# ZhaoyangLyu/Point_Diffusion_Refinement

Measured on AMD Instinct MI355X. Metric: DDPM reverse steps/sec (T=1000, N=2048), higher is better.
Workload: dtype f32; 1 GPU; BASELINE configs[1]: B=32/GPU, N=2048, 3072-pt mirrored condition, T=1000 DDPM reverse sampling, random-init dual-path PointNet++ (9.76 M params), cached condition step; global_batch=32, parallelism=dp1, launch=hipGraph replay, noise=device Philox, execution=fused channel-last HIP

## Files before the change

### point_diffusion_refinement_amd/csrc/ball_query.hip

```cpp
#include "pdr_common.h"

namespace {

template <int NCH, bool RESIDENT>
__global__ __launch_bounds__(256) void ball_query_kernel(
    const float* __restrict__ new_xyz, const float* __restrict__ xyz, int n, int m,
    float radius2, int nsample, int qpw, int* __restrict__ idx,
    int* __restrict__ counts) {
  const int b = blockIdx.y;
  const int lane = threadIdx.x & 63;
  const int wave = __builtin_amdgcn_readfirstlane(threadIdx.x >> 6);
  const float* p = xyz + static_cast<size_t>(b) * n * 3;
  const float* q = new_xyz + static_cast<size_t>(b) * m * 3;
  int* oi = idx + static_cast<size_t>(b) * m * nsample;
  int* oc = counts + static_cast<size_t>(b) * m;

  const int nch = RESIDENT ? NCH : (n + 63) / 64;
  float px[NCH], py[NCH], pz[NCH];
  if constexpr (RESIDENT) {
    if constexpr (NCH <= 32) {
#pragma unroll
      for (int c = 0; c < NCH; ++c) {
        const int k = min(c * 64 + lane, n - 1);
        px[c] = p[k * 3 + 0];
        py[c] = p[k * 3 + 1];
        pz[c] = p[k * 3 + 2];
      }
#pragma unroll
      for (int c = 0; c < NCH; ++c) {
        const bool ok = c * 64 + lane < n;
        px[c] = ok ? px[c] : __builtin_inff();
        py[c] = ok ? py[c] : __builtin_inff();
        pz[c] = ok ? pz[c] : __builtin_inff();
      }
    } else {
#pragma unroll
      for (int c = 0; c < NCH; ++c) {
        const int k = c * 64 + lane;
        const bool ok = k < n;
        px[c] = ok ? p[k * 3 + 0] : __builtin_inff();
        py[c] = ok ? p[k * 3 + 1] : __builtin_inff();
        pz[c] = ok ? p[k * 3 + 2] : __builtin_inff();
      }
    }
    __builtin_amdgcn_s_waitcnt(0x0F70);
  }

  const int j0 = (blockIdx.x * 4 + wave) * qpw;
  const int jf = min(j0, m - 1);
  float nqx = q[jf * 3 + 0], nqy = q[jf * 3 + 1], nqz = q[jf * 3 + 2];
  for (int jj = 0; jj < qpw; ++jj) {
    const int j = j0 + jj;
    if (j >= m) break;
    const float qx = nqx, qy = nqy, qz = nqz;
    {
      const int jn = min(j + 1, m - 1);
      nqx = q[jn * 3 + 0], nqy = q[jn * 3 + 1], nqz = q[jn * 3 + 2];
    }
    int* row = oi + static_cast<size_t>(j) * nsample;
    int cnt = 0;
    int first = 0;
    auto scan = [&](int c, float x, float y, float z) {
      const float dx = qx - x, dy = qy - y, dz = qz - z;
      const float d2 = PDR_SUM3(dx, dy, dz);
      const bool hit = d2 < radius2;
      const unsigned long long mask = __ballot(hit);
      if (mask != 0ull) {
        if (cnt == 0) first = c * 64 + __builtin_ctzll(mask);
        const int pos = cnt + __builtin_amdgcn_mbcnt_hi(
                                  static_cast<unsigned>(mask >> 32),
                                  __builtin_amdgcn_mbcnt_lo(static_cast<unsigned>(mask), 0u));
        if (hit && pos < nsample) row[pos] = c * 64 + lane;
        cnt += __builtin_popcountll(mask);
      }
    };
    if constexpr (RESIDENT) {
#pragma unroll
      for (int c = 0; c < NCH; ++c) {
        if (cnt < nsample) scan(c, px[c], py[c], pz[c]);
      }
    } else {
      for (int c = 0; c < nch && cnt < nsample; ++c) {
        const int k = c * 64 + lane;
        const bool ok = k < n;
        const int kc = ok ? k : n - 1;
        const float x = p[kc * 3 + 0], y = p[kc * 3 + 1], z = p[kc * 3 + 2];
        scan(c, ok ? x : __builtin_inff(), ok ? y : __builtin_inff(), ok ? z : __builtin_inff());
      }
    }
    const int filled = cnt < nsample ? cnt : nsample;
    for (int l = filled + lane; l < nsample; l += 64) row[l] = first;
    if (lane == 0) oc[j] = filled;
  }
}

struct BallPlan {
  int nch;
  int resident;
  int qpw;
  int gx;
};

int plan_ball_query(int B, int n, int m, BallPlan* p) {
  if (B < 0 || n <= 0 || m < 0) return PDR_EINVAL;
  p->nch = p->resident = p->qpw = p->gx = 0;
  if (B == 0 || m == 0) return PDR_OK;
  constexpr int kResident[] = {1, 2, 4, 8, 16, 32, 48, 64};
  p->nch = 1;
  for (const int nch : kResident)
    if (n <= 64 * nch) {
      p->nch = nch, p->resident = 1;
      break;
    }
  int qpw = 16;
  while (qpw > 1 && static_cast<long long>(B) * ((m + 4 * qpw - 1) / (4 * qpw)) < 1024) qpw >>= 1;
  p->qpw = qpw;
  p->gx = (m + 4 * qpw - 1) / (4 * qpw);
  return PDR_OK;
}

template <int NCH, bool RESIDENT>
int launch(const BallPlan& p, const float* new_xyz, const float* xyz, int B, int n, int m, float radius2,
           int nsample, int* idx, int* counts, hipStream_t s) {
  hipLaunchKernelGGL((ball_query_kernel<NCH, RESIDENT>), dim3(p.gx, B), dim3(256), 0, s, new_xyz, xyz, n,
                     m, radius2, nsample, p.qpw, idx, counts);
  return pdr::check_launch();
}

}

extern "C" int pdr_ball_query_plan(int B, int n, int m, int out[4]) {
  if (!out) return PDR_EINVAL;
  BallPlan p;
  const int rc = plan_ball_query(B, n, m, &p);
  if (rc != PDR_OK) return rc;
  out[0] = p.nch, out[1] = p.resident, out[2] = p.qpw, out[3] = p.gx;
  return PDR_OK;
}

extern "C" int pdr_ball_query(const float* new_xyz, const float* xyz, int B, int n, int m,
                              float radius, int nsample, int* idx, int* counts,
                              pdr_stream_t stream) {
  BallPlan p;
  const int rc = plan_ball_query(B, n, m, &p);
  if (rc != PDR_OK) return rc;
  if (nsample <= 0) return PDR_EINVAL;
  if (B == 0 || m == 0) return PDR_OK;
  if (!new_xyz || !xyz || !idx || !counts) return PDR_EINVAL;
  hipStream_t s = pdr::as_stream(stream);
  const float radius2 = radius * radius;
  if (!p.resident) return launch<1, false>(p, new_xyz, xyz, B, n, m, radius2, nsample, idx, counts, s);
#define PDR_BQ_CASE(NCH) \
  case NCH:              \
    return launch<NCH, true>(p, new_xyz, xyz, B, n, m, radius2, nsample, idx, counts, s)
  switch (p.nch) {
    PDR_BQ_CASE(1);
    PDR_BQ_CASE(2);
    PDR_BQ_CASE(4);
    PDR_BQ_CASE(8);
    PDR_BQ_CASE(16);
    PDR_BQ_CASE(32);
    PDR_BQ_CASE(48);
    PDR_BQ_CASE(64);
  }
#undef PDR_BQ_CASE
  return PDR_EUNSUPPORTED;
}
```

### point_diffusion_refinement_amd/pointnet2/fused_network.py

```python
import contextlib
import ctypes
from collections import namedtuple

import torch
import torch.nn as nn
import torch.nn.functional as F

from .. import _lib
from ..pointnet2_ops import _ext
from ..pointnet2_ops.attention import MyGroupNorm
from .models.pointnet2_ssg_sem import calc_t_emb


USE_SPLIT_FIRST = True
SPLIT_QUERY_CONV = True
FUSE_SCORE_POOL = True
FUSE_CONDITION_BRANCH = True
USE_VIRTUAL_FIRST = True
USE_VIRTUAL_KNN = True
GATHER_RES = 4096
GATHER_RES_KNN = True
NATIVE_EMBED = True
STEP_TABLE = True
FUSE_GLOBAL_PNET = True
# ... 1453 lines not shown
        if self.s1[0][1] is None or self.s2[0][1] is None:
            raise NotImplementedError("fused Pnet2Stage: the first layer of a stage is normalised")

    @staticmethod
    def _mlp(x, stages, B, n):
        (c1, n1), (c2, n2) = stages
        lo = run_layer(x, c1, fold=FoldReq(n1, c1.Cout, n))
        a1 = act_from(lo, c1.Cout, B * n, B, n, scale=lo.folded[0], shift=lo.folded[1], post_relu=True)
        if n2 is None:
            return act_from(run_layer(a1, c2), c2.Cout, B * n, B, n)
        lo = run_layer(a1, c2, fold=FoldReq(n2, c2.Cout, n))
        return act_from(lo, c2.Cout, B * n, B, n, scale=lo.folded[0], shift=lo.folded[1], post_relu=True)

    def __call__(self, g_in):
        B, n, _ = g_in.shape
        x = Act(feature_segments(g_in), B * n, B, n)
        f = self._mlp(x, self.s1, B, n)
        g = act_colmax(f)
        C1 = f.C
        Y, ld = f.segs[0].t, f.segs[0].ld
        dev = g.device
        one = torch.ones((B, C1), device=dev) if f.scale is None else f.scale
        zero = torch.zeros((B, C1), device=dev)
        tm = _lib.load().pdr_fused_layer_tile_rows(n, self.s2[0][0].Cout)
        d = 1
        while d * 2 <= tm and n % (d * 2) == 0 and tm % (d * 2) == 0:
            d *= 2
        if d > 1 and C1 % 4 == 0:
            second, s_second = Seg(torch.zeros((B * n // d, C1), device=dev), 0, C1, C1, d), one
        else:
            second, s_second = Seg(Y, 0, C1, ld), zero
        both = Act([Seg(Y, 0, C1, ld), second], B * n, B, n,
                   scale=torch.cat([one, s_second], 1).contiguous(),
                   shift=torch.cat([zero if f.shift is None else f.shift, zero], 1).contiguous(),
                   add=torch.cat([zero, g], 1).contiguous(), add_ld=2 * C1, post_relu=f.post_relu)
        return act_colmax(self._mlp(both, self.s2, B, n))


class FusedCloudConditionNet:

    def __init__(self, net, precision="f32"):
        hp = net.hparams
        if precision == "split_bf16":
            import warnings
            warnings.warn("precision='split_bf16' is a deprecated alias of 'split_f16' (f16 hi + lo halves; see the "
                          "range contract in include/pdr_hip.h)", DeprecationWarning, stacklevel=2)
            precision = "split_f16"
        if precision not in ("f32", "split_f16"):
            raise ValueError("precision must be 'f32' or 'split_f16'")
        self.precision = precision
        if net.scale_factor != 1:
            raise NotImplementedError("fused path: scale_factor == 1 (coordinates are not rescaled here)")
        if not (net.include_local_feature and net.include_global_feature and hp['include_class_condition']
                and net.attach_position_to_input_feature and net.bn and not hp['bn_first']
                and net.network_activation == 'relu'):
            raise NotImplementedError("configuration outside the fused family (see module docstring)")
        self.net = net
        self.bank = EmbeddingBank()
        b = self.bank
        self.enc_map = [FusedGroupedBlock(m.mapper, m.mlp, m.attention_module, b) for m in net.encoder_feature_map]
        self.dec_map = [FusedGroupedBlock(m.mapper, m.mlp, m.attention_module, b) for m in net.decoder_feature_map]
        self.sa = []
        for sa in net.SA_modules:
            if len(sa.groupers) != 1 or not sa.use_attention_module:
                raise NotImplementedError("fused path: single-scale SA with attention")
            blk = FusedGroupedBlock(sa.groupers[0], sa.mlps[0], sa.attention_modules[0], b)
            blk.npoint = sa.npoint
            self.sa.append(blk)
        self.fp = [FusedKnnFP(fp, b) for fp in net.FP_modules]
        for blk in self.enc_map + self.dec_map + self.sa:
            blk.dedup = True
        self.cond_sa = []
        for sa in net.SA_modules_condition:
            if len(sa.groupers) != 1 or not sa.use_attention_module:
                raise NotImplementedError("fused path: single-scale SA with attention")
            blk = FusedGroupedBlock(sa.groupers[0], sa.mlps[0], sa.attention_modules[0], b)
            blk.npoint = sa.npoint
            self.cond_sa.append(blk)
        self.cond_fp = [FusedKnnFP(fp, b) for fp in net.FP_modules_condition]
        head = list(net.fc_lyaer)
        if not (len(head) == 4 and isinstance(head[1], nn.GroupNorm) and isinstance(head[2], nn.ReLU)):
            raise NotImplementedError("fused path: Conv1d -> GroupNorm -> ReLU -> Conv1d head")
        self.head1, self.head_norm, self.head2 = Conv([head[0]]), Norm(head[1]), Conv([head[3]])
        b.pack()
        try:
            self.global_pnet = FusedPnet2Stage(net.global_pnet)
        except NotImplementedError:
            self.global_pnet = None
        self.enc_cl = self.dec_cl = None
        self._synced = False
        self._streams = {"side": None, "fps": None, "aux": None}
        self.return_strided_eps = False
        self.two_streams = True
        self._label_key = None
        self.dedup = True
        self.probe = None
        self.step_table = None

    def _stream_named(self, name):
        if self._streams[name] is None:
            self._streams[name] = torch.cuda.Stream(device=next(self.net.parameters()).device)
        return self._streams[name]

    def sync_condition(self):
        net = self.net

        def convert(dst, src):
            if dst is not None and len(dst) == len(src) and all(d.shape == (f.shape[0], f.shape[2], f.shape[1])
                                                                for d, f in zip(dst, src)):
                for d, f in zip(dst, src):
                    d.copy_(f.transpose(1, 2))
                return dst
            return [f.transpose(1, 2).contiguous() for f in src]

        self.enc_cl = convert(self.enc_cl, net.encoder_cond_features)
        self.dec_cl = convert(self.dec_cl, net.decoder_cond_features)
        saved_precision = _PRECISION[0]
        _PRECISION[0] = self.precision
        with torch.no_grad():
            _new_forward()
            for i, blk in enumerate(self.enc_map):
                blk.prepare_static_source(net.l_uvw[i], self.enc_cl[i])
            for i, blk in enumerate(self.dec_map):
                blk.prepare_static_source(net.l_uvw[i], self.dec_cl[i])
            _XYZ4.clear()
            self.bank.evaluate_kind("c", net.global_feature, static=True)
        _PRECISION[0] = saved_precision
        self._synced = True

    def _condition_branch(self, condition):
        net, bank = self.net, self.bank
        uvw = condition[:, :, 0:3].contiguous()
        cond0 = torch.cat([condition[:, :, 3:], uvw / net.scale_factor], dim=2).contiguous() \
            if condition.shape[2] > 3 else (uvw / net.scale_factor)
        raw = net.partial_in_fea_dim - 3 if net.attach_position_to_input_feature else net.partial_in_fea_dim
        g_in = torch.cat([uvw, condition[:, :, 3:3 + raw]], dim=2) if raw > 0 else uvw
        if self.global_pnet is not None and FUSE_GLOBAL_PNET:
            net.global_feature = self.global_pnet(g_in.contiguous())
        else:
            net.global_feature = net.global_pnet(g_in.transpose(1, 2)).detach().clone()
        l_uvw, l_cond = [uvw], [cond0]
        for i, sa in enumerate(self.cond_sa):
            sel = _ext.furthest_point_sampling(l_uvw[i], sa.npoint)
            l_uvw.append(gather_rows(l_uvw[i], sel))
            centre = gather_rows(l_cond[i], sel)
            l_cond.append(sa(l_uvw[i], l_cond[i], l_uvw[i + 1], centre, bank, subset=True))
        net.l_uvw = l_uvw
        net.encoder_cond_features = [f.transpose(1, 2).contiguous() for f in l_cond]
        for i in range(-1, -(len(self.cond_fp) + 1), -1):
            l_cond[i - 1] = self.cond_fp[i](l_uvw[i - 1], l_uvw[i], l_cond[i - 1], l_cond[i], bank)
        net.decoder_cond_features = [f.transpose(1, 2).contiguous() for f in l_cond]
        self._synced = False

    @torch.no_grad()
    def forward(self, pointcloud, condition, ts=None, label=None, use_retained_condition_feature=False):
        net, hp, bank = self.net, self.net.hparams, self.bank
        fresh = not use_retained_condition_feature or net.encoder_cond_features is None or \
            net.decoder_cond_features is None or net.global_feature is None
        if fresh:
            if not FUSE_CONDITION_BRANCH:
                out = net(pointcloud, condition, ts=ts, label=label,
                          use_retained_condition_feature=use_retained_condition_feature)
                if use_retained_condition_feature and label is not None:
                    self._refresh_class_embedding(label)
                return out
        saved = _PRECISION[0], _NET_DEDUP[0], _PROBE[0]
        _PRECISION[0], _NET_DEDUP[0], _PROBE[0] = self.precision, bool(self.dedup), self.probe
        saved_par = _PAR["stream"]
        _PAR["stream"] = self._stream_named("aux") if self.two_streams else None
        try:
            if fresh:
                _new_forward()
                self._condition_branch(condition)
            return self._forward_cached(pointcloud, condition, ts, label)
        finally:
            _PRECISION[0], _NET_DEDUP[0], _PROBE[0] = saved
            _PAR["stream"] = saved_par
            if not use_retained_condition_feature:
                self.reset_cond_features()

    def _embeddings(self, ts, label):
        net, hp, bank = self.net, self.net.hparams, self.bank
        if ts is not None and hp['include_t']:
            if STEP_TABLE and self.step_table is not None and self._embed_select(ts.shape[0]):
                pass
            elif not (NATIVE_EMBED and ts.is_cuda and "t" in bank.W and self._embed_linear_chain(ts)):
                t_emb = net.activation(net.fc_t1(calc_t_emb(ts, hp['t_dim'])))
                t_emb = net.activation(net.fc_t2(t_emb))
                bank.evaluate_kind("t", t_emb)
        if self._label_key is None or self._label_key[0] is not label or self._label_key[1] != label._version \
                or "c2" not in bank.out:
            self._refresh_class_embedding(label)
        if "c" not in bank.out:
            bank.evaluate_kind("c", net.global_feature, static=True)

    def _refresh_class_embedding(self, label):
        with torch.no_grad():
            self.bank.evaluate_kind("c2", self.net.class_emb(label), static=True)
        self._label_key = (label, label._version)

    def build_step_table(self, ts_values):
        bank = self.bank
        if not (STEP_TABLE and NATIVE_EMBED and self.net.hparams['include_t'] and "t" in bank.W and ts_values.is_cuda):
            return None
        saved = bank.out.get("t")
        ok = self._embed_linear_chain(ts_values.float().contiguous())
        table = bank.out.get("t") if ok else None
        if saved is not None:
            bank.out["t"] = saved
        elif "t" in bank.out:
            del bank.out["t"]
        if table is None or table.shape[1] % 4 != 0:
            return None
        return table

    def _embed_select(self, B):
        table, t_dev = self.step_table
        out = torch.empty((B, table.shape[1]), dtype=torch.float32, device=table.device)
        rc = _lib.load().pdr_embed_select(table.data_ptr(), table.shape[1], table.shape[0], t_dev.data_ptr(), B,
                                          table.shape[1], out.data_ptr(), out.shape[1], _stream())
        if rc == _lib.PDR_EUNSUPPORTED:
            return False
        _lib.check(rc, "embed_select")
        self.bank.out["t"] = out
        return True

    def _embed_linear_chain(self, ts):
        net, bank, lib = self.net, self.bank, _lib.load()
        t_dim = net.hparams['t_dim']
        if t_dim % 8 != 0 or ts.dim() != 1:
            return False
        if ts.dtype != torch.float32:
            ts = ts.float()
        from .models.pointnet2_ssg_sem import _frequencies
        B, half = ts.shape[0], t_dim // 2
        freq = _frequencies(half, ts.device)
        dev = ts.device
        h1 = torch.empty((B, 4 * t_dim), dtype=torch.float32, device=dev)
        h2 = torch.empty((B, 4 * t_dim), dtype=torch.float32, device=dev)
        Wb, bb = bank.W["t"], bank.b["t"]
        out = torch.empty((B, Wb.shape[0]), dtype=torch.float32, device=dev)
        w1, w2 = net.fc_t1.weight, net.fc_t2.weight
        st = _stream()
        rc = lib.pdr_embed_linear(None, 0, ts.data_ptr(), ts.stride(0), freq.data_ptr(), half, w1.data_ptr(),
                                  net.fc_t1.bias.data_ptr(), B, t_dim, 4 * t_dim, 1, h1.data_ptr(), h1.shape[1], st)
        if rc == _lib.PDR_EUNSUPPORTED:
            return False
        _lib.check(rc, "embed_linear")
        _lib.check(lib.pdr_embed_linear(h1.data_ptr(), h1.shape[1], None, 0, None, 0, w2.data_ptr(),
                                        net.fc_t2.bias.data_ptr(), B, 4 * t_dim, 4 * t_dim, 1, h2.data_ptr(),
                                        h2.shape[1], st), "embed_linear")
        _lib.check(lib.pdr_embed_linear(h2.data_ptr(), h2.shape[1], None, 0, None, 0, Wb.data_ptr(), bb.data_ptr(), B,
                                        4 * t_dim, Wb.shape[0], 0, out.data_ptr(), out.shape[1], st), "embed_linear")
        bank.out["t"] = out
        return True

    def _forward_cached(self, pointcloud, condition, ts, label):
        net, hp, bank = self.net, self.net.hparams, self.bank
        B, N, _ = pointcloud.shape
        _new_forward()
        mark("step:begin")
        xyz = pointcloud[:, :, 0:3].contiguous()
        feat0 = torch.cat([pointcloud[:, :, 3:], xyz], dim=2).contiguous() if pointcloud.shape[2] > 3 else xyz
        if not self._synced:
            self.sync_condition()
        enc_cl, dec_cl = self.enc_cl, self.dec_cl
        l_uvw = net.l_uvw

        main = torch.cuda.current_stream()
        side = self._stream_named("side")
        fps_on = FPS_STREAM and _dedup_on()
        hoist0_main = HOIST_LEVEL0_ON_MAIN and _dedup_on()
        fps_s = self._stream_named("fps") if fps_on else side
        xyz4(xyz)
        side.wait_stream(main)
        fps_s.wait_stream(main)
        nlev = len(self.sa)
        l_xyz, sels, fm_neigh, sa_neigh, knn, tables = [xyz], [], {}, [None] * nlev, {}, {}
        ev_fps, ev_sa, ev_fm = [None] * nlev, [None] * nlev, {}
        side_tables_on = SIDE_TABLES and USE_SPLIT_FIRST

        def fm_key(i, blk):
            return (i % (nlev + 1), blk.radius, blk.nsample)

        def event(stream):
            ev = torch.cuda.Event()
            ev.record(stream)
            return ev

        def sample_level(i):
            with torch.cuda.stream(fps_s):
                sel = _ext.furthest_point_sampling(l_xyz[i], self.sa[i].npoint)
                sels.append(sel)
                l_xyz.append(gather_rows(l_xyz[i], sel))
                ev_fps[i] = event(fps_s)

        def transfer_level(lv, tables_for):
            with torch.cuda.stream(side):
                for blk in ([self.enc_map[lv]] if lv < nlev else []) + [self.dec_map[lv]]:
                    if fm_key(lv, blk) not in fm_neigh:
                        fm_neigh[fm_key(lv, blk)] = blk.plan_ahead(blk.neighbours(l_uvw[lv], l_xyz[lv]), l_xyz[lv])
                    if side_tables_on and blk.split is not None and blk in tables_for:
                        tables[id(blk)] = blk.side_tables(fm_neigh[fm_key(lv, blk)], l_xyz[lv], True)
                ev_fm[lv] = event(side)

        def group_level(i):
            sa = self.sa[i]
            if not fps_on:
                sample_level(i)
            with torch.cuda.stream(side):
                if fps_on:
                    side.wait_event(ev_fps[i])
                sa_neigh[i] = sa.plan_ahead(sa.neighbours(l_xyz[i], l_xyz[i + 1]), l_xyz[i + 1])
                xyz4(l_xyz[i + 1])
                if side_tables_on and sa.split is not None:
                    tables[id(sa)] = sa.side_tables(sa_neigh[i], l_xyz[i + 1], False)
                ev_sa[i] = event(side)

        with torch.cuda.stream(fps_s):
            mark("fps:begin")
        if fps_on:
            sample_level(0)
        transfer_level(0, (self.enc_map[0], self.dec_map[0]) if hoist0_main else (self.enc_map[0],))
        with torch.cuda.stream(side):
            mark("side:first_ball_query_done")
        if fps_on:
            for i in range(1, nlev):
                sample_level(i)

        mark("main:before_embeddings", detail=True)
        self._embeddings(ts, label)
        mark("main:embeddings_done")
        ev_emb = event(main)

        def transfer(blk, l, cl, query, V2=None, q_ahead=None):
            prep = prepared.get(id(blk))
            if prep is not None:
                if prep.event is not None:
                    main.wait_event(prep.event)
                return blk.finish(prep, query)
            return blk(l_uvw[l], cl[l], l_xyz[l], query, bank, subset=False, neigh=fm_neigh[fm_key(l, blk)], V2=V2,
                       q_ahead=q_ahead)

        prepared = {}
        hoist = AHEAD_DECODER_MAPS and USE_SPLIT_FIRST and self.two_streams
        hoisted = [False]
        hoist_enc = AHEAD_ENCODER_MAPS and hoist and (_dedup_on() or AHEAD_ENCODER_MAPS_WHOLE)

        def hoist_map(blk, cl, l):
            if tables.get(id(blk)) is None:
                return
            with torch.cuda.stream(side):
                if not hoisted[0]:
                    side.wait_event(ev_emb)
                    hoisted[0] = True
                with _single_stream():
                    prep = blk.prepare(l_uvw[l], cl[l], l_xyz[l], bank, subset=False, neigh=fm_neigh[fm_key(l, blk)],
                                       V2=tables[id(blk)])
                prepared[id(blk)] = prep._replace(event=event(side))

        def geometry_tail():
            with torch.cuda.stream(side):
                mark("side:encoder_geometry_done")
                if side_tables_on:
                    if self.dec_map[0].split is not None and id(self.dec_map[0]) not in tables:
                        tables[id(self.dec_map[0])] = self.dec_map[0].side_tables(fm_neigh[fm_key(0, self.dec_map[0])],
                                                                                  l_xyz[0], True)
                    for i in range(-1, -(len(self.fp) + 1), -1):
                        fp = self.fp[i]
                        if fp.split is not None:
                            tables[id(fp)] = QueryTables(fp.split.query_tables(l_xyz[i - 1], has_v0=False))
                for i in range(-1, -(len(self.fp) + 1), -1):
                    knn[i] = _ext.knn_group(l_xyz[i - 1], l_xyz[i], self.fp[i].K)
                mark("side:knn_done")
                return event(side)

        for k in range(nlev):
            group_level(k)
            lv = k + 1
            transfer_level(lv, (self.enc_map[lv],) if lv < nlev else (self.dec_map[lv],))
            if lv < nlev and hoist_enc:
                hoist_map(self.enc_map[lv], enc_cl, lv)
        if side_tables_on:
            with torch.cuda.stream(side):
                for l in range(1, nlev):
                    blk = self.dec_map[l]
                    if blk.split is not None and id(blk) not in tables:
                        tables[id(blk)] = blk.side_tables(fm_neigh[fm_key(l, blk)], l_xyz[l], True)
        ev_knn = geometry_tail()
        if hoist:
            for l in range(nlev, 0 if hoist0_main else -1, -1):
                hoist_map(self.dec_map[l], dec_cl, l)

        def table_early(split, Cm, early_feats, src_xyz):
            aux = _PAR["stream"]
            if not (SPLIT_SOURCE_TABLES and USE_SPLIT_FIRST and aux is not None) or early_feats.shape[2] % 4 != 0:
                return None
            aux.wait_event(event(main))
            with torch.cuda.stream(aux):
                part = split.source_table_early(Cm, early_feats, src_xyz)
                return part, event(aux)

        def table_late(split, pending, late_feats):
            if pending is None:
                return None
            main.wait_event(pending[1])
            return split.source_table_late(late_feats, pending[0])

        q0 = None
        if QUERY_CONV_AHEAD and SPLIT_QUERY_CONV and QUERIES_IN_PLACE and USE_SPLIT_FIRST and _PAR["stream"] is not None:
            q0 = _ready(self.enc_map[0].att.query_conv(feat0.reshape(B * N, -1), B, N))
        main.wait_event(ev_fm[0])
        mark("main:after_wait_first_ball_query")
        l_feat = [feat0]
        for i, sa in enumerate(self.sa):
            if i > 0:
                main.wait_event(ev_fm[i])
            Cm = self.enc_map[i].att.D
            pend = table_early(sa._make_split(Cm + l_feat[i].shape[2]), Cm, l_feat[i], l_xyz[i]) if i > 0 else None
            mapped = transfer(self.enc_map[i], i, enc_cl, l_feat[i], V2=tables.get(id(self.enc_map[i])),
                              q_ahead=q0 if i == 0 else None)
            mark("main:enc_map%d_done" % i)
            if i == 0 and hoist0_main and hoist and tables.get(id(self.dec_map[0])) is not None:
                with _single_stream():
                    prepared[id(self.dec_map[0])] = self.dec_map[0].prepare(
                        l_uvw[0], dec_cl[0], l_xyz[0], bank, subset=False, neigh=fm_neigh[fm_key(0, self.dec_map[0])],
                        V2=tables.get(id(self.dec_map[0])))
            sa_in = Cat(mapped, l_feat[i]) if USE_SPLIT_FIRST else torch.cat([mapped, l_feat[i]], dim=2)
            U_ahead = table_late(sa.split, pend, mapped)
            if i == 0 and SA0_TABLE_AHEAD and USE_SPLIT_FIRST and hoist0_main and _PAR["stream"] is not None:
                U_ahead = sa._make_split(sa_in.shape[2]).source_table(sa_in, l_xyz[i])
            main.wait_event(ev_sa[i])
            mark("main:after_wait_sa%d_geometry" % i)
            centre = gather_rows(sa_in, sels[i])
            l_feat.append(sa(l_xyz[i], sa_in, l_xyz[i + 1], centre, bank, subset=True, neigh=sa_neigh[i],
                             V2=tables.get(id(sa)), U=U_ahead))
            mark("main:sa%d_done" % i)
        main.wait_event(ev_knn)
        for i in range(-1, -(len(self.fp) + 1), -1):
            Cm = self.dec_map[i].att.D
            pend = table_early(self.fp[i]._make_split(Cm + l_feat[i].shape[2]), Cm, l_feat[i], l_xyz[i]) \
                if USE_SPLIT_FIRST else None
            mapped = transfer(self.dec_map[i], i % (nlev + 1), dec_cl, l_feat[i], V2=tables.get(id(self.dec_map[i])))
            fp_in = Cat(mapped, l_feat[i]) if USE_SPLIT_FIRST else torch.cat([mapped, l_feat[i]], dim=2)
            mark("main:dec_map%d_done" % (i % (nlev + 1)))
            l_feat[i - 1] = self.fp[i](l_xyz[i - 1], l_xyz[i], l_feat[i - 1], fp_in, bank, knn=knn[i],
                                       V2=tables.get(id(self.fp[i])), U=table_late(self.fp[i].split, pend, mapped))
            mark("main:fp%d_done" % (i % (nlev + 1)))
        mapped = transfer(self.dec_map[0], 0, dec_cl, l_feat[0], V2=tables.get(id(self.dec_map[0])))
        Cm, Cf = mapped.shape[2], l_feat[0].shape[2]
        head_in = Act([Seg(mapped, 0, Cm, Cm), Seg(l_feat[0], 0, Cf, Cf), Seg(xyz4(xyz), 0, 3, 4)], B * N, B, N)
        lo = run_layer(head_in, self.head1, fold=FoldReq(self.head_norm, self.head1.Cout, N))
        out = run_layer(act_from(lo, self.head1.Cout, B * N, B, N, scale=lo.folded[0], shift=lo.folded[1],
                                 post_relu=True), self.head2).Y
        mark("main:head_done")
        eps = out.view(B, N, out.shape[1])[:, :, :self.head2.Cout]
        return eps if self.return_strided_eps else eps.contiguous()

    __call__ = forward

    def reset_cond_features(self):
        self.net.reset_cond_features()
        self._synced = False
        self._label_key = None

    def parameters(self):
        return self.net.parameters()
```

Measured before the change: 6090 cloud-steps/s.

## Reject far queries by cloud bounding box and pair-vectorise ball-query scan

The ball-query kernel now loads one query per lane, computes the cloud's axis-aligned bounding box with a wave reduction, and skips any query whose box distance exceeds a conservatively rounded-up radius. Skipped queries get a zero count and a zero-filled row. The remaining queries are scanned with float2 packed distance math, batching several ballots per group, and large clouds are staged through shared memory. Separately, the first level's encoder neighbour event is recorded before the decoder tables are built, so the main stream can start enc_map0 earlier. This adds more registers and control complexity in exchange for fewer wasted scans and less serialisation.

After: 6081 cloud-steps/s. About the same (-0.2%).

```diff
diff --git a/point_diffusion_refinement_amd/csrc/ball_query.hip b/point_diffusion_refinement_amd/csrc/ball_query.hip
--- a/point_diffusion_refinement_amd/csrc/ball_query.hip
+++ b/point_diffusion_refinement_amd/csrc/ball_query.hip
@@ -1,11 +1,15 @@
+#include <type_traits>
+
 #include "pdr_common.h"
 
 namespace {
+
+typedef float bq_f2 __attribute__((ext_vector_type(2)));
 
 template <int NCH, bool RESIDENT>
 __global__ __launch_bounds__(256) void ball_query_kernel(
     const float* __restrict__ new_xyz, const float* __restrict__ xyz, int n, int m,
-    float radius2, int nsample, int qpw, int* __restrict__ idx,
+    float radius2, float r_up, int nsample, int qpw, int* __restrict__ idx,
     int* __restrict__ counts) {
   const int b = blockIdx.y;
   const int lane = threadIdx.x & 63;
@@ -15,77 +19,152 @@
   int* oi = idx + static_cast<size_t>(b) * m * nsample;
   int* oc = counts + static_cast<size_t>(b) * m;
 
-  const int nch = RESIDENT ? NCH : (n + 63) / 64;
-  float px[NCH], py[NCH], pz[NCH];
+  const int j0 = (blockIdx.x * 4 + wave) * qpw;
+  const int jl = j0 + lane;
+  const bool mine = lane < qpw && jl < m;
+  float qlx, qly, qlz;
+  {
+    const int jc = min(jl, m - 1);
+    qlx = q[jc * 3 + 0], qly = q[jc * 3 + 1], qlz = q[jc * 3 + 2];
+  }
+
+  constexpr int NP = (NCH + 1) / 2;
+  const int np = RESIDENT ? NP : (n + 127) / 128;
+  bq_f2 px[NP], py[NP], pz[NP];
+  if constexpr (RESIDENT && NCH <= 16) {
+#pragma unroll
+    for (int c = 0; c < NCH; ++c) {
+      const int k = min(c * 64 + lane, n - 1);
+      px[c >> 1][c & 1] = p[k * 3 + 0];
+      py[c >> 1][c & 1] = p[k * 3 + 1];
+      pz[c >> 1][c & 1] = p[k * 3 + 2];
+    }
+  } else if constexpr (RESIDENT) {
+    __shared__ float cloud[NCH * 64 * 3];
+    constexpr int T = (NCH * 64 * 3 + 255) / 256;
+    const int nf = n * 3;
+    float stage[T];
+#pragma unroll
+    for (int t = 0; t < T; ++t) {
+      const int i = t * 256 + static_cast<int>(threadIdx.x);
+      stage[t] = p[min(i, nf - 1)];
+    }
+#pragma unroll
+    for (int t = 0; t < T; ++t) {
+      const int i = t * 256 + static_cast<int>(threadIdx.x);
+      if (i < nf) cloud[i] = stage[t];
+    }
+    __syncthreads();
+#pragma unroll
+    for (int c = 0; c < NCH; ++c) {
+      const int k = min(c * 64 + lane, n - 1);
+      px[c >> 1][c & 1] = cloud[k * 3 + 0];
+      py[c >> 1][c & 1] = cloud[k * 3 + 1];
+      pz[c >> 1][c & 1] = cloud[k * 3 + 2];
+    }
+  }
+
+  float lox = __builtin_inff(), loy = __builtin_inff(), loz = __builtin_inff();
+  float hix = -__builtin_inff(), hiy = -__builtin_inff(), hiz = -__builtin_inff();
   if constexpr (RESIDENT) {
-    if constexpr (NCH <= 32) {
-#pragma unroll
-      for (int c = 0; c < NCH; ++c) {
-        const int k = min(c * 64 + lane, n - 1);
-        px[c] = p[k * 3 + 0];
-        py[c] = p[k * 3 + 1];
-        pz[c] = p[k * 3 + 2];
-      }
-#pragma unroll
-      for (int c = 0; c < NCH; ++c) {
-        const bool ok = c * 64 + lane < n;
-        px[c] = ok ? px[c] : __builtin_inff();
-        py[c] = ok ? py[c] : __builtin_inff();
-        pz[c] = ok ? pz[c] : __builtin_inff();
-      }
-    } else {
-#pragma unroll
-      for (int c = 0; c < NCH; ++c) {
-        const int k = c * 64 + lane;
-        const bool ok = k < n;
-        px[c] = ok ? p[k * 3 + 0] : __builtin_inff();
-        py[c] = ok ? p[k * 3 + 1] : __builtin_inff();
-        pz[c] = ok ? p[k * 3 + 2] : __builtin_inff();
-      }
-    }
-    __builtin_amdgcn_s_waitcnt(0x0F70);
-  }
-
-  const int j0 = (blockIdx.x * 4 + wave) * qpw;
-  const int jf = min(j0, m - 1);
-  float nqx = q[jf * 3 + 0], nqy = q[jf * 3 + 1], nqz = q[jf * 3 + 2];
-  for (int jj = 0; jj < qpw; ++jj) {
-    const int j = j0 + jj;
-    if (j >= m) break;
-    const float qx = nqx, qy = nqy, qz = nqz;
-    {
-      const int jn = min(j + 1, m - 1);
-      nqx = q[jn * 3 + 0], nqy = q[jn * 3 + 1], nqz = q[jn * 3 + 2];
-    }
+#pragma unroll
+    for (int c = 0; c < NCH; ++c) {
+      const float x = px[c >> 1][c & 1], y = py[c >> 1][c & 1], z = pz[c >> 1][c & 1];
+      lox = fminf(lox, x), loy = fminf(loy, y), loz = fminf(loz, z);
+      hix = fmaxf(hix, x), hiy = fmaxf(hiy, y), hiz = fmaxf(hiz, z);
+    }
+#pragma unroll
+    for (int off = 32; off >= 1; off >>= 1) {
+      lox = fminf(lox, __shfl_xor(lox, off, 64)), hix = fmaxf(hix, __shfl_xor(hix, off, 64));
+      loy = fminf(loy, __shfl_xor(loy, off, 64)), hiy = fmaxf(hiy, __shfl_xor(hiy, off, 64));
+      loz = fminf(loz, __shfl_xor(loz, off, 64)), hiz = fmaxf(hiz, __shfl_xor(hiz, off, 64));
+    }
+    __builtin_amdgcn_sched_barrier(0);
+#pragma unroll
+    for (int c = 0; c < 2 * NP; ++c) {
+      const bool ok = c < NCH && c * 64 + lane < n;
+      px[c >> 1][c & 1] = ok ? px[c >> 1][c & 1] : __builtin_inff();
+      py[c >> 1][c & 1] = ok ? py[c >> 1][c & 1] : __builtin_inff();
+      pz[c >> 1][c & 1] = ok ? pz[c >> 1][c & 1] : __builtin_inff();
+    }
+  }
+
+  unsigned live;
+  {
+    bool out = false;
+    if constexpr (RESIDENT)
+      out = (lox - qlx > r_up) | (qlx - hix > r_up) | (loy - qly > r_up) | (qly - hiy > r_up) | (loz - qlz > r_up) |
+            (qlz - hiz > r_up);
+    live = static_cast<unsigned>(__ballot(mine && !out));
+    unsigned skip = static_cast<unsigned>(__ballot(mine && out));
+    if (mine && out) oc[jl] = 0;
+    while (skip != 0u) {
+      int* row = oi + static_cast<size_t>(j0 + __builtin_ctz(skip)) * nsample;
+      skip &= skip - 1u;
+      for (int l = lane; l < nsample; l += 64) row[l] = 0;
+    }
+  }
+
+  auto uniform = [](float v, int l) {
+    return __builtin_bit_cast(float, __builtin_amdgcn_readlane(__builtin_bit_cast(int, v), l));
+  };
+  while (live != 0u) {
+    const int ql = __builtin_ctz(live);
+    live &= live - 1u;
+    const int j = j0 + ql;
+    const float sx = uniform(qlx, ql), sy = uniform(qly, ql), sz = uniform(qlz, ql);
+    const bq_f2 qx = {sx, sx}, qy = {sy, sy}, qz = {sz, sz};
     int* row = oi + static_cast<size_t>(j) * nsample;
     int cnt = 0;
     int first = 0;
-    auto scan = [&](int c, float x, float y, float z) {
-      const float dx = qx - x, dy = qy - y, dz = qz - z;
-      const float d2 = PDR_SUM3(dx, dy, dz);
-      const bool hit = d2 < radius2;
-      const unsigned long long mask = __ballot(hit);
-      if (mask != 0ull) {
-        if (cnt == 0) first = c * 64 + __builtin_ctzll(mask);
-        const int pos = cnt + __builtin_amdgcn_mbcnt_hi(
-                                  static_cast<unsigned>(mask >> 32),
-                                  __builtin_amdgcn_mbcnt_lo(static_cast<unsigned>(mask), 0u));
-        if (hit && pos < nsample) row[pos] = c * 64 + lane;
-        cnt += __builtin_popcountll(mask);
+    auto take = [&](int c, bool hit, unsigned long long mask) {
+      if (cnt == 0) first = c * 64 + __builtin_ctzll(mask);
+      const int pos = cnt + __builtin_amdgcn_mbcnt_hi(static_cast<unsigned>(mask >> 32),
+                                                      __builtin_amdgcn_mbcnt_lo(static_cast<unsigned>(mask), 0u));
+      if (hit && pos < nsample) row[pos] = c * 64 + lane;
+      cnt += __builtin_popcountll(mask);
+    };
+    auto scan = [&](auto gc, int k0, const bq_f2* x, const bq_f2* y, const bq_f2* z) {
+      constexpr int G = decltype(gc)::value;
+      bool hit[2 * G];
+      unsigned long long mask[2 * G], any = 0ull;
+#pragma unroll
+      for (int g = 0; g < G; ++g) {
+        const bq_f2 dx = qx - x[g], dy = qy - y[g], dz = qz - z[g];
+        const bq_f2 d2 = __builtin_elementwise_fma(dz, dz, __builtin_elementwise_fma(dx, dx, dy * dy));
+#pragma unroll
+        for (int h = 0; h < 2; ++h) {
+          hit[2 * g + h] = d2[h] < radius2;
+          mask[2 * g + h] = __ballot(hit[2 * g + h]);
+          any |= mask[2 * g + h];
+        }
+      }
+      if (any != 0ull) {
+#pragma unroll
+        for (int h = 0; h < 2 * G; ++h)
+          if (mask[h] != 0ull && cnt < nsample) take(2 * k0 + h, hit[h], mask[h]);
       }
     };
     if constexpr (RESIDENT) {
-#pragma unroll
-      for (int c = 0; c < NCH; ++c) {
-        if (cnt < nsample) scan(c, px[c], py[c], pz[c]);
+      constexpr int G = NP % 4 == 0 ? 4 : NP;
+      static_assert(NP % G == 0 && G <= 4, "the pairs of an instantiation split into whole groups");
+#pragma unroll
+      for (int k = 0; k < NP; k += G) {
+        if (cnt < nsample) scan(std::integral_constant<int, G>(), k, px + k, py + k, pz + k);
       }
     } else {
-      for (int c = 0; c < nch && cnt < nsample; ++c) {
-        const int k = c * 64 + lane;
-        const bool ok = k < n;
-        const int kc = ok ? k : n - 1;
-        const float x = p[kc * 3 + 0], y = p[kc * 3 + 1], z = p[kc * 3 + 2];
-        scan(c, ok ? x : __builtin_inff(), ok ? y : __builtin_inff(), ok ? z : __builtin_inff());
+      for (int k = 0; k < np && cnt < nsample; ++k) {
+        bq_f2 x, y, z;
+#pragma unroll
+        for (int h = 0; h < 2; ++h) {
+          const int i = (2 * k + h) * 64 + lane;
+          const bool ok = i < n;
+          const int ic = ok ? i : n - 1;
+          x[h] = ok ? p[ic * 3 + 0] : __builtin_inff();
+          y[h] = ok ? p[ic * 3 + 1] : __builtin_inff();
+          z[h] = ok ? p[ic * 3 + 2] : __builtin_inff();
+        }
+        scan(std::integral_constant<int, 1>(), k, &x, &y, &z);
       }
     }
     const int filled = cnt < nsample ? cnt : nsample;
@@ -119,11 +198,17 @@
   return PDR_OK;
 }
 
+float reject_radius(float radius2) {
+  float r = sqrtf(radius2);
+  while (r * r < radius2) r = nextafterf(r, __builtin_inff());
+  return r;
+}
+
 template <int NCH, bool RESIDENT>
 int launch(const BallPlan& p, const float* new_xyz, const float* xyz, int B, int n, int m, float radius2,
            int nsample, int* idx, int* counts, hipStream_t s) {
   hipLaunchKernelGGL((ball_query_kernel<NCH, RESIDENT>), dim3(p.gx, B), dim3(256), 0, s, new_xyz, xyz, n,
-                     m, radius2, nsample, p.qpw, idx, counts);
+                     m, radius2, reject_radius(radius2), nsample, p.qpw, idx, counts);
   return pdr::check_launch();
 }
 
diff --git a/point_diffusion_refinement_amd/pointnet2/fused_network.py b/point_diffusion_refinement_amd/pointnet2/fused_network.py
--- a/point_diffusion_refinement_amd/pointnet2/fused_network.py
+++ b/point_diffusion_refinement_amd/pointnet2/fused_network.py
@@ -1779,7 +1779,9 @@
                         fm_neigh[fm_key(lv, blk)] = blk.plan_ahead(blk.neighbours(l_uvw[lv], l_xyz[lv]), l_xyz[lv])
                     if side_tables_on and blk.split is not None and blk in tables_for:
                         tables[id(blk)] = blk.side_tables(fm_neigh[fm_key(lv, blk)], l_xyz[lv], True)
-                ev_fm[lv] = event(side)
+                    if lv == 0 and blk is self.enc_map[0]:
+                        ev_fm[lv] = event(side)
+                ev_fm["dec0" if lv == 0 else lv] = event(side)
 
         def group_level(i):
             sa = self.sa[i]
@@ -1898,6 +1900,8 @@
             mapped = transfer(self.enc_map[i], i, enc_cl, l_feat[i], V2=tables.get(id(self.enc_map[i])),
                               q_ahead=q0 if i == 0 else None)
             mark("main:enc_map%d_done" % i)
+            if i == 0:
+                main.wait_event(ev_fm["dec0"])
             if i == 0 and hoist0_main and hoist and tables.get(id(self.dec_map[0])) is not None:
                 with _single_stream():
                     prepared[id(self.dec_map[0])] = self.dec_map[0].prepare(
```
